# nlaha/genomics-rs

Measured on AMD Instinct MI355X. Metric: GCUPS (DP cell updates/s) at 30k×30k NW, 1/2/4/8 MI355X; % HBM roofline, higher is better.
Workload: dtype int16x2 (two pairs per register, exact, relative to int32 block bases)

## Files before the change

genomics-rs_amd/csrc/gx_api.h:

```cpp
#pragma once
#include <hip/hip_runtime.h>
#include <immintrin.h>

#include <algorithm>
#include <atomic>
#include <chrono>
#include <climits>
#include <condition_variable>
#include <functional>
#include <cstdio>
#include <cstdlib>
#include <cstring>
#include <memory>
#include <mutex>
#include <new>
#include <string>
#include <thread>
#include <vector>

#include "../../include/gx.h"
#include "gx_internal.h"

#pragma GCC visibility push(hidden)

// ... 206 lines not shown
    std::vector<DevBuf> free_list;
    std::vector<std::vector<uint8_t>> st_s1, st_s2;
    DevBuf st_chars;
    std::vector<size_t> st_off1, st_off2;
    SmallAlpha st_alpha;
    std::vector<Walk> walk_cache;
    TbOut tb_cache;
    PinnedBuf tb_pin;
    PinnedBuf io_pin;
    WorkPool workers;
    struct Slot {
        PinnedBuf fpin, tjpin, tbpin;
        hipEvent_t fb = nullptr, fe = nullptr, tb = nullptr, te = nullptr, fdone = nullptr, tdone = nullptr;
        hipEvent_t fres = nullptr;
        DevBuf held_pres;
        TbOut out;
        DevBuf held[4];
        void* tjob = nullptr;
        size_t tjob_cap = 0;
        std::vector<TbDev> tjob_last;
        void* fdesc = nullptr;
        size_t fdesc_cap = 0;
        std::vector<char> fdesc_last;
    } slots[4];
    int last_lay = 0, last_W = 0, last_pbytes = 0;
    int last_pbits = 0;
    int last_chunks = 1;
    int last_twin = 0;
    int last_rows = 0;
    int last_tbl = 0;
    int last_groups = 1;
    DevBuf sums_dev;
    unsigned long long* sums_dst = nullptr;
    std::vector<uint64_t> sums_host;
    bool pass_rec = false;
    size_t pass_off = 0, pass_P = 0;
    int pass_k = 0;
    std::vector<gx_result> pass_res;
    std::shared_ptr<struct KeptFill> kept;
    bool keep_capture = false;
    HostScores kept_hs{};
    Scores32 kept_sc{};
    uint64_t cmp_gpu = 0, cmp_host = 0, cmp_ovf = 0, cmp_levels = 0;
    uint64_t cmp_batches = 0;
    uint64_t cmp_cells = 0;
    double cmp_run_ms = 0.0;
    uint64_t suf_rounds = 0, suf_passes = 0;
    uint64_t suf_digit_passes[8] = {};
    double suf_sort_ms = 0.0, suf_lcp_ms = 0.0, suf_fold_ms = 0.0;
    uint64_t srch_words = 0;
    double srch_ms = 0.0, srch_locate_ms = 0.0;
};

struct PairHost {
// ... 8 lines not shown
    bool lcs_rows = false;
    size_t ltrace_off = 0, ltrace_bytes = 0;
    bool pairs_borrowed = false;
    bool pres_held = false;
    std::vector<PairDev> pd;
    std::vector<PairRes> res;
    int W = 4;
    int lay = 0;
    int slot = -1;
    PairRes* pin_res = nullptr;
    int* pin_status = nullptr;
    int total_bands = 0, total_strips = 0;
    bool planes_on = false, lcs_on = false, track_on = false;
    bool d8 = false;
    bool shift = false;
    bool twin = false;
    int rows = kRowsPerLane;
    bool w16 = false;
    bool nocodes = false;
    bool noskel = false;
    bool local_on = false;
    hipStream_t stream = nullptr;
    bool plan_only = false;
    bool table = false;
    int g = 0;
    double fill_ms = 0.0;
    bool wide = false;
    DevBuf wrows, wdesc, wres_d;
    std::vector<WideDev> wd;
    std::vector<WideRes> wres;
};

inline int job_strip_rows(const FillJob& j) { return j.twin && j.lay == 0 ? kWave * j.rows : strip_rows(j.lay); }

struct KeptFill {
    gx_context* ctx = nullptr;
    FillJob job;
    std::vector<int> dev_of;
    ~KeptFill();
};

static size_t align_up(size_t x, size_t a) { return (x + a - 1) / a * a; }


struct gx_table {
    gx_context* ctx = nullptr;
// ... 122 lines not shown
int run_fill_wide(gx_context* ctx, const std::vector<std::pair<const uint8_t*, const uint8_t*>>& proc,
                  const std::vector<PairHost>& ph, const HostScores& hs, int is_local, bool planes, bool track,
                  bool lcs, FillJob& job);
hipError_t enqueue_plane_sums(gx_context* ctx, const FillJob& job, const Scores32& sc,
                              unsigned long long* out, hipStream_t st = nullptr);

StartIn start_in(const FillJob& job, size_t p);
StartIn start_in(const PairRes& r);
int label_boundary(const HostScores& hs, int is_local, const uint8_t* s1, size_t n, const uint8_t* s2,
                   size_t m, uint64_t i, uint64_t j, int last, Walk& w);
int label_walk_records(const HostScores& hs, int is_local, const uint8_t* s1, size_t n, const uint8_t* s2,
                       size_t m, uint64_t si, uint64_t sj, const TbOut& tb, size_t p, Walk& w);
int run_traceback(gx_context* ctx, const std::vector<const FillJob*>& jv, const std::vector<TbStart>& starts,
                  TbOut& out, int slot, bool collect, bool dev_end_E, hipStream_t ts);
int run_traceback(gx_context* ctx, const FillJob& job, const std::vector<TbStart>& starts, TbOut& out,
                  int slot = -1, bool collect = true, bool dev_end_E = false);
int tb_collect(gx_context* ctx, int slot, size_t P, TbOut& out);
int start_cell_common(const HostScores& hs, int is_local, size_t n, size_t m, const StartIn& r,
                      uint64_t* si, uint64_t* sj, int64_t* score);
int copy_steps(const Walk& w, gx_step* steps, size_t cap);
int label_batch(gx_context* ctx, const std::vector<PairHost>& ph, const HostScores& hs, int is_local, bool track,
                const std::vector<int>& dev_of, const std::vector<uint64_t>& si,
                const std::vector<uint64_t>& sj, const std::vector<int64_t>& score,
                const std::vector<PairRes>& res, const TbOut& tb, double fill_ms, std::vector<Walk>& walks);

int batch_core_wide(gx_context* ctx, const std::vector<PairHost>& ph,
                    const std::vector<std::pair<const uint8_t*, const uint8_t*>>& proc, const HostScores& hs,
                    int is_local, bool planes, bool track, std::vector<Walk>& walks, double* fill_ms);
int batch_core_steps(gx_context* ctx, const std::vector<PairHost>& ph,
                     const std::vector<std::pair<const uint8_t*, const uint8_t*>>& proc, const HostScores& hs,
                     const Scores32& sc, int is_local, bool planes, bool track, int nsteps,
                     std::vector<Walk>& walks, double* fill_ms, const uint8_t* chars_dev,
                     const std::vector<size_t>* off1, const std::vector<size_t>* off2,
                     const SmallAlpha* staged_alpha, const PassSet* alt = nullptr);

struct SufInfo {
    uint64_t rounds = 0, passes = 0;
    uint64_t digit_passes[8] = {};
    double sort_ms = 0, lcp_ms = 0, fold_ms = 0;
};
struct SufDev {
    DevBuf text, k[2], v[2], rank, flags, table, tmp, small, fold, bwt;
    int cur = 0;
    uint64_t h = 8;
    uint64_t* pin = nullptr;
    void release(gx_context* ctx) {
        for (DevBuf* b : {&text, &k[0], &k[1], &v[0], &v[1], &rank, &flags, &table, &tmp, &small, &fold, &bwt})
            pool_put(ctx, *b);
    }
};
int suffix_device_sa(gx_context* ctx, const uint8_t* t, uint32_t N, bool with_stats, bool with_bwt, SufDev& w,
// ... 52 lines not shown
```

genomics-rs_amd/csrc/gx_api_batch.cpp:

```cpp
#include "gx_api.h"

int batch_core_wide(gx_context* ctx, const std::vector<PairHost>& ph,
                    const std::vector<std::pair<const uint8_t*, const uint8_t*>>& proc, const HostScores& hs,
                    int is_local, bool planes, bool track, std::vector<Walk>& walks, double* fill_ms) {
    const size_t P = ph.size();
    std::vector<size_t> idx;
    for (size_t p = 0; p < P; ++p) if (ph[p].n >= 1 && ph[p].m >= 1) idx.push_back(p);
    std::vector<PairHost> dph;
    std::vector<std::pair<const uint8_t*, const uint8_t*>> dproc;
    for (size_t p : idx) { dph.push_back(ph[p]); dproc.push_back(proc[p]); }
    FillJob job;
    std::vector<PairRes> res(P, PairRes{});
    std::vector<StartIn> sin(P, StartIn{0, 0, 0, 0});
    std::vector<uint64_t> si(P), sj(P);
    std::vector<int64_t> score(P);
    TbOut& tb = ctx->tb_cache;
    tb.ms = 0;
    int rc = GX_OK;
    if (!idx.empty()) {
        rc = run_fill_wide(ctx, dproc, dph, hs, is_local, planes, track, false, job);
        if (rc) { job_release(ctx, job); return rc; }
        for (size_t k = 0; k < idx.size(); ++k) { res[idx[k]] = job.res[k]; sin[idx[k]] = start_in(job, k); }
    }
    for (size_t p = 0; p < P; ++p) start_cell_common(hs, is_local, ph[p].n, ph[p].m, sin[p], &si[p], &sj[p], &score[p]);
// ... 77 lines not shown
        for (size_t k = 0; k < idx.size(); ++k) kdev[idx[k]] = (int)k;
        keep_job(ctx, job, kdev);
    }
    struct PhaseLog {
        clk::time_point c0, c1, c2;
        double fill_ms, tb_ms;
        size_t P;
        ~PhaseLog() {
            const char* e = getenv("GX_LOG");
            if (!e || strcmp(e, "debug")) return;
            auto ms = [](clk::time_point a, clk::time_point b) {
                return std::chrono::duration<double, std::milli>(b - a).count();
            };
            fprintf(stderr, "[gx DEBUG] batch P=%zu fill %.3f ms (kernel %.3f) traceback %.3f ms (kernel %.3f) "
                            "label %.3f ms\n", P, ms(c0, c1), fill_ms, ms(c1, c2), tb_ms, ms(c2, clk::now()));
        }
    } plog{c0, c1, c2, job.fill_ms, tb.ms, P};
    std::vector<int> dev_of(P, -1);
    for (size_t k = 0; k < idx.size(); ++k) dev_of[idx[k]] = (int)k;
    return label_batch(ctx, ph, hs, is_local, track, dev_of, si, sj, score, res, tb, job.fill_ms, walks);
}

static constexpr int kOverlapNo = -1000;
static int batch_core_overlap(gx_context* ctx, const std::vector<PairHost>& ph,
                              const std::vector<std::pair<const uint8_t*, const uint8_t*>>& proc, const HostScores& hs,
                              const Scores32& sc, int is_local, bool planes, int nsteps, std::vector<Walk>& walks, double* fill_ms,
                              const uint8_t* chars_dev, const std::vector<size_t>* off1,
                              const std::vector<size_t>* off2, const SmallAlpha& alpha,
                              const std::vector<size_t>& idx, const PassSet* alt) {
    const size_t P = ph.size(), Q = idx.size();
    size_t G = std::max<size_t>(2, (is_local ? Q / 5 : (Q + 1) / 2) & ~(size_t)1);
    if (const char* e = getenv("GX_OVERLAP_A"); e && atoi(e) >= 2 && (size_t)atoi(e) + 2 <= Q)
        G = (size_t)atoi(e) & ~(size_t)1;
    std::vector<size_t> gi[2];
    gi[0].assign(idx.begin(), idx.begin() + (long)G);
    gi[1].assign(idx.begin() + (long)G, idx.end());
    const std::vector<PairHost>* const PH[2] = {&ph, alt ? alt->ph : &ph};
    const std::vector<std::pair<const uint8_t*, const uint8_t*>>* const PR[2] = {&proc, alt ? alt->proc : &proc};
    const std::vector<size_t>* const O1[2] = {off1, alt ? alt->off1 : off1};
    const std::vector<size_t>* const O2[2] = {off2, alt ? alt->off2 : off2};
    std::vector<Walk>* const WK[2] = {&walks, alt ? alt->walks : &walks};
    const size_t poff[2] = {ctx->pass_off, alt ? alt->pass_off : ctx->pass_off};
    std::vector<PairHost> dph[2][2];
    std::vector<std::pair<const uint8_t*, const uint8_t*>> dproc[2][2];
    std::vector<size_t> o1[2][2], o2[2][2];
    for (int v = 0; v < 2; ++v)
// ... 22 lines not shown
    auto fill = [&](int g, int k) {
        FillJob& j = g == 0 ? jA[k & 1] : jB;
        j.stream = g == 0 ? sA : sB;
        const int v = k & 1;
        return run_fill(ctx, dproc[v][g], dph[v][g], sc, is_local, planes, false, false, j, chars_dev,
                        chars_dev ? &o1[v][g] : nullptr, chars_dev ? &o2[v][g] : nullptr, &alpha, 2 * g + (k & 1), false);
    };
    auto trace = [&](int k) {
        HIPCHK(hipStreamWaitEvent(sT, ctx->slots[k & 1].fdone, 0));
        HIPCHK(hipStreamWaitEvent(sT, ctx->slots[2 + (k & 1)].fdone, 0));
        return run_traceback(ctx, std::vector<const FillJob*>{&jA[k & 1], &jB}, starts, ctx->slots[k & 1].out, k & 1,
                             false, is_local != 0, sT);
    };
    auto take = [&](const FillJob& j, const std::vector<size_t>& g) {
        for (size_t q = 0; q < g.size(); ++q) res[g[q]] = j.res[q];
    };
    auto drain = [&]() {
        (void)hipStreamSynchronize(sA); (void)hipStreamSynchronize(sB); (void)hipStreamSynchronize(sT);
        (void)hipStreamSynchronize(ctx->cstream);
        for (auto& j : jA) job_release(ctx, j);
        job_release(ctx, jB);
        release_slots(ctx);
    };
    {
        FillJob pa, pb;
        pa.plan_only = pb.plan_only = true;
        int prc = run_fill(ctx, dproc[0][0], dph[0][0], sc, is_local, planes, false, false, pa, chars_dev,
                           chars_dev ? &o1[0][0] : nullptr, chars_dev ? &o2[0][0] : nullptr, &alpha, 0, false);
        if (!prc)
            prc = run_fill(ctx, dproc[0][1], dph[0][1], sc, is_local, planes, false, false, pb, chars_dev,
                           chars_dev ? &o1[0][1] : nullptr, chars_dev ? &o2[0][1] : nullptr, &alpha, 2, false);
        if (prc || !(pa.noskel && pb.noskel && pa.twin && pb.twin && pa.lay == pb.lay && pa.rows == pb.rows)) return kOverlapNo;
    }
    unsigned long long* const sums0 = ctx->sums_dst;
    HIPCHK(hipEventRecord(ctx->ev0, sA));
    int rc = fill(0, 0);
    if (!rc) { rc = fill(1, 0); jb_live = !rc; }
    if (!rc && !(jA[0].noskel && jB.noskel && jA[0].lay == jB.lay && jA[0].twin && jB.twin && jA[0].rows == jB.rows)) {
        drain();
        ctx->sums_dst = sums0;
        return kOverlapNo;
    }
    if (!rc) rc = trace(0);
    for (int k = 0; k < nsteps && !rc; ++k) {
        const int a = k & 1;
        if (k + 1 < nsteps) {
            if ((rc = fill(0, k + 1))) break;
            if ((rc = fill_collect(ctx, jB))) break;
            take(jB, gi[1]);
            job_release(ctx, jB);
            HIPCHK(hipStreamWaitEvent(sB, ctx->slots[a].te, 0));
            if ((rc = fill(1, k + 1))) break;
            if (k + 2 == nsteps) {
                HIPCHK(hipStreamWaitEvent(sB, ctx->slots[(k + 1) & 1].fdone, 0));
                HIPCHK(hipEventRecord(ctx->ev1, sB));
            }
            if (!(jA[(k + 1) & 1].noskel && jB.noskel)) { rc = fail(GX_EHIP, "overlapped batch: fill formats changed"); break; }
// ... 4 lines not shown
        }
        if ((rc = fill_collect(ctx, jA[a]))) break;
        take(jA[a], gi[0]);
        if (k + 1 == nsteps) {
            HIPCHK(hipEventSynchronize(ctx->ev1));
            float ms = 0.f;
            HIPCHK(hipEventElapsedTime(&ms, ctx->ev0, ctx->ev1));
            fsum = ms;
        }
        if ((rc = tb_collect(ctx, a, Q, ctx->slots[a].out))) break;
        job_release(ctx, jA[a]);
        for (size_t p = 0; p < P; ++p)
            start_cell_common(hs, is_local, ph[p].n, ph[p].m, start_in(res[p]), &si[p], &sj[p], &score[p]);
        ctx->pass_off = poff[a];
        if ((rc = label_batch(ctx, *PH[a], hs, is_local, false, dev_of, si, sj, score, res, ctx->slots[a].out,
                              jA[a].fill_ms + jB.fill_ms, *WK[a])))
            break;
    }
    drain();
    (void)jb_live;
    ctx->pass_off = poff[0];
    if (rc) return rc;
    ctx->last_groups = 2;
    if (fill_ms) *fill_ms = fsum / nsteps;
    return GX_OK;
}

int batch_core_steps(gx_context* ctx, const std::vector<PairHost>& ph,
                     const std::vector<std::pair<const uint8_t*, const uint8_t*>>& proc, const HostScores& hs,
                     const Scores32& sc, int is_local, bool planes, bool track, int nsteps,
                     std::vector<Walk>& walks, double* fill_ms, const uint8_t* chars_dev,
                     const std::vector<size_t>* off1, const std::vector<size_t>* off2,
                     const SmallAlpha* staged_alpha, const PassSet* alt) {
    const size_t P = ph.size();
    ctx->last_groups = 1;
    std::vector<size_t> idx;
    for (size_t p = 0; p < P; ++p) if (ph[p].n >= 1 && ph[p].m >= 1) idx.push_back(p);
    const std::vector<PairHost>* const PH[2] = {&ph, alt ? alt->ph : &ph};
    const std::vector<std::pair<const uint8_t*, const uint8_t*>>* const PR[2] = {&proc, alt ? alt->proc : &proc};
    const std::vector<size_t>* const O1[2] = {off1, alt ? alt->off1 : off1};
    const std::vector<size_t>* const O2[2] = {off2, alt ? alt->off2 : off2};
    std::vector<Walk>* const WK[2] = {&walks, alt ? alt->walks : &walks};
    const size_t poff[2] = {ctx->pass_off, alt ? alt->pass_off : ctx->pass_off};
    struct OffBack {
        gx_context* c;
        size_t v;
        ~OffBack() { c->pass_off = v; }
    } off_back{ctx, poff[0]};
    if (nsteps <= 1 || idx.empty() || getenv("GX_TRACE_FILE")) {
        double f = 0, fsum = 0;
        for (int s = 0; s < std::max(nsteps, 1); ++s) {
            const int v = s & 1;
            ctx->pass_off = poff[v];
            const int rc = batch_core(ctx, *PH[v], *PR[v], hs, sc, is_local, planes, track, *WK[v], &f, chars_dev,
                                      O1[v], O2[v], staged_alpha);
            if (rc) return rc;
            fsum += f;
        }
// ... 302 lines not shown
```

genomics-rs_amd/csrc/gx_api_context.cpp:

```cpp
#include "gx_api.h"


thread_local std::string g_err;
int fail(int code, const std::string& msg) {
    g_err = msg;
    return code;
}

int gx_internal_fail(int code, const std::string& msg) { return fail(code, msg); }

extern "C" const char* gx_last_error(void) { return g_err.c_str(); }
extern "C" const char* gx_version(void) { return "genomics-rs_amd 0.1 (gfx950)"; }

bool log_info() {
    static int v = -1;
    if (v < 0) {
        const char* e = getenv("GX_LOG");
        v = (e && (!strcmp(e, "info") || !strcmp(e, "debug"))) ? 1 : 0;
    }
    return v == 1;
}

void* pinned_grow(PinnedBuf& b, size_t bytes) {
    if (b.cap < bytes) {
// ... 143 lines not shown
        for (PinnedBuf* b : {&s.fpin, &s.tjpin, &s.tbpin})
            if (b->p) (void)hipHostFree(b->p);
        for (hipEvent_t e : {s.fb, s.fe, s.tb, s.te, s.fdone, s.tdone, s.fres})
            if (e) (void)hipEventDestroy(e);
        if (s.tjob) (void)hipFree(s.tjob);
        if (s.fdesc) (void)hipFree(s.fdesc);
    }
    if (ctx->ev0) (void)hipEventDestroy(ctx->ev0);
    if (ctx->ev1) (void)hipEventDestroy(ctx->ev1);
    if (ctx->ev2) (void)hipEventDestroy(ctx->ev2);
    if (ctx->stream) (void)hipStreamDestroy(ctx->stream);
    if (ctx->cstream) (void)hipStreamDestroy(ctx->cstream);
    if (ctx->stream2) (void)hipStreamDestroy(ctx->stream2);
    if (ctx->tstream) (void)hipStreamDestroy(ctx->tstream);
    if (ctx->pstream) (void)hipStreamDestroy(ctx->pstream);
    delete ctx;
}

void release_held(gx_context* ctx, int slot) {
    for (DevBuf& b : ctx->slots[slot].held) { pool_put(ctx, b); b = DevBuf{}; }
}
void release_slots(gx_context* ctx) {
    (void)hipStreamSynchronize(ctx->cstream);
    for (int k = 0; k < 4; ++k) {
        release_held(ctx, k);
        pool_put(ctx, ctx->slots[k].held_pres);
    }
}
```

genomics-rs_amd/csrc/gx_api_fill.cpp:

```cpp
#include "gx_api.h"

void unshift_results(FillJob& j) {
    if (!j.shift) return;
    for (size_t p = 0; p < j.res.size() && p < j.pd.size(); ++p)
        if (j.pd[p].n >= 1 && j.pd[p].m >= 1) j.res[p].end_SM += (j.pd[p].n + j.pd[p].m) * j.g;
}

void job_release(gx_context* ctx, FillJob& j) {
    if (j.pairs_borrowed) { j.pairs = DevBuf{}; j.pairs_borrowed = false; }
    if (j.pres_held) { j.pres = DevBuf{}; j.pres_held = false; }
    pool_put(ctx, j.chars); pool_put(ctx, j.planes); pool_put(ctx, j.codes); pool_put(ctx, j.feed);
    pool_put(ctx, j.progress); pool_put(ctx, j.sres); pool_put(ctx, j.pres); pool_put(ctx, j.pairs);
    pool_put(ctx, j.counter); pool_put(ctx, j.skel); pool_put(ctx, j.ccodes);
    pool_put(ctx, j.wrows); pool_put(ctx, j.wdesc); pool_put(ctx, j.wres_d); pool_put(ctx, j.lcs);
}

void release_or_hold(gx_context* ctx, FillJob& j, bool last_pass, bool* held) {
    if (ctx->keep_capture && last_pass) { *held = true; return; }
    job_release(ctx, j);
}
void keep_job(gx_context* ctx, FillJob& j, const std::vector<int>& dev_of) {
    auto k = std::make_shared<KeptFill>();
    k->ctx = ctx;
    k->dev_of = dev_of;
// ... 44 lines not shown
    if (twin && is_local) {
        const int K = std::max(0, -std::min(sc.sm, sc.smm));
        scl.koff = K; scl.sm = sc.sm + K; scl.smm = sc.smm + K;
    }
    const bool w16 = tp.w16;
    job.w16 = w16;
    job.nocodes = w16;
    job.noskel = job.nocodes;
    const int rows = tp.rows;
    job.rows = rows;
    const int SRf = twin ? kWave * rows : SR;
    const bool twin_tbl = twin && tbl && (!planes || w16) && scl.sm >= 0 && scl.sm <= 255 && scl.smm >= 0 &&
                          scl.smm <= 255;
    ctx->last_twin = twin ? 1 : 0;
    ctx->last_rows = twin ? rows : 0;
    ctx->last_tbl = (twin ? twin_tbl : tbl) ? 1 : 0;
    const int Wf = twin ? Wt : W;
    const size_t plane_esz = d8 ? 1 : sizeof(int32_t);
    job.W = Wf;
    ctx->last_lay = cs2 ? 2 : lay; ctx->last_W = Wf;
    ctx->last_pbytes = planes ? (w16 ? 2 : (int)(plane_esz * 3)) : 0;
    ctx->last_pbits = planes ? (w16 ? 12 : (int)(plane_esz * 24)) : 0;
    const size_t P = ph.size();
    if (job.plan_only) { job.twin = twin; return GX_OK; }
    job.pd.assign(P, PairDev{});
    size_t chars_bytes = 0, plane_elems = 0, code_elems = 0, feed_recs = 0, prog_elems = 0, skel_elems = 0;
    std::vector<size_t> c1o(P), c2o(P), po(P), co(P), fo(P), gofs(P), so(P);
    int bands = 0, strips = 0;
    std::vector<int> mate(P, -1), half(P, 0);
    if (twin)
        for (const auto& t : tw) {
            mate[t.first] = t.second; mate[t.second] = t.first;
            half[t.first] = 0;
            if (t.second != t.first) half[t.second] = 1;
        }
    for (size_t p = 0; p < P; ++p) {
        const int n = (int)ph[p].n, m = (int)ph[p].m;
        PairDev& d = job.pd[p];
        d.n = n; d.m = m;
        int ns = n, ms = m;
        if (twin) {
            const PairHost& y = ph[mate[p]];
            ns = (int)std::max(ph[p].n, y.n); ms = (int)std::max(ph[p].m, y.m);
        }
        d.strips = ceil_div(ns, SRf);
        d.bands = ceil_div(d.strips, Wf);
        d.rows = twin ? rows : 0;
// ... 12 lines not shown
        if (!twin) {
            d.band_base = bands;
            bands += d.bands;
            so[p] = skel_elems; skel_elems += (size_t)d.strips * d.skel_stride;
            fo[p] = feed_recs; feed_recs += (size_t)std::max(d.bands - 1, 0) * d.feed_stride;
            gofs[p] = prog_elems; prog_elems += (size_t)std::max(d.bands - 1, 0) * kProgStride;
        }
    }
    if (twin)
        for (const auto& t : tw) {
            PairDev& d = job.pd[t.first];
            const size_t a = t.first, b = t.second;
            d.band_base = bands; job.pd[b].band_base = bands;
            bands += d.bands;
            so[a] = so[b] = skel_elems; skel_elems += (size_t)d.strips * d.skel_stride;
            fo[a] = fo[b] = feed_recs; feed_recs += (size_t)std::max(d.bands - 1, 0) * d.feed_stride * 2;
            gofs[a] = gofs[b] = prog_elems; prog_elems += (size_t)std::max(d.bands - 1, 0) * kProgStride;
            if (w16) { po[a] = po[b] = plane_elems; plane_elems += (size_t)d.strips * d.t4 * w12_group_bytes(rows); }
        }
    job.total_bands = bands;
    job.total_strips = strips;
    int rc;
    const int nplanes = w16 ? 1 : (lcs && !job.lcs_rows) ? 4 : 3;
    if (!chars_dev) {
        if ((rc = pool_get(ctx, chars_bytes, &job.chars, fs))) return rc;
    }
    if (planes && (rc = pool_get(ctx, plane_elems * plane_esz * nplanes, &job.planes, fs))) return rc;
    const bool want_codes = codes && !job.nocodes;
    if (want_codes && (rc = pool_get(ctx, code_elems * sizeof(uint32_t), &job.codes, fs))) return rc;
    if ((rc = pool_get(ctx, std::max<size_t>(skel_elems, 1) * sizeof(int), &job.skel, fs))) return rc;
    if ((rc = pool_get(ctx, std::max<size_t>(feed_recs, 1) * sizeof(Rec), &job.feed, fs))) return rc;
    if ((rc = pool_get(ctx, std::max(strips, 1) * sizeof(StripRes), &job.sres, fs))) return rc;
    if (getenv("GX_LCS_ALONE"))
        HIPCHK(hipMemsetAsync(job.sres.p, 0, std::max(strips, 1) * sizeof(StripRes), fs));
    const size_t res_bytes = P * sizeof(PairRes), prog_bytes = std::max<size_t>(prog_elems, 1) * sizeof(int);
    if ((rc = pool_get(ctx, res_bytes + 64 + prog_bytes, &job.pres, fs))) return rc;
    int* const counter = (int*)((char*)job.pres.p + res_bytes);
    int* const progress = counter + 16;
    std::vector<int> order;
    order.reserve(2 * (size_t)bands);
    if (twin) {
        int maxb = 0;
        for (const auto& t : tw) maxb = std::max(maxb, job.pd[t.first].bands);
        for (int lb = 0; lb < maxb; ++lb)
            for (size_t q = 0; q < tw.size(); ++q)
                if (lb < job.pd[tw[q].first].bands) { order.push_back((int)q); order.push_back(lb); }
        for (const auto& t : tw) { order.push_back(t.first); order.push_back(t.second); }
    } else {
        int maxb = 0;
        for (size_t p = 0; p < P; ++p) maxb = std::max(maxb, job.pd[p].bands);
// ... 364 lines not shown
```

genomics-rs_amd/csrc/gx_api_walk.cpp:

```cpp
#include "gx_api.h"

StartIn start_in(const FillJob& job, size_t p) {
    if (job.wide) return StartIn{job.wres[p].end_SM, job.wres[p].lmax_val, (uint64_t)job.wres[p].lmax_i,
                                 (uint64_t)job.wres[p].lmax_j};
    const PairRes& r = job.res[p];
    return StartIn{r.end_SM, r.lmax_val, (uint64_t)r.lmax_i, (uint64_t)r.lmax_j};
}
StartIn start_in(const PairRes& r) { return StartIn{r.end_SM, r.lmax_val, (uint64_t)r.lmax_i, (uint64_t)r.lmax_j}; }

int label_boundary(const HostScores& hs, int is_local, const uint8_t* s1, size_t n, const uint8_t* s2,
                   size_t m, uint64_t i, uint64_t j, int last, Walk& w) {
    gx_result& r = w.res;
    for (;;) {
        int64_t I, D, S;
        boundary_cell(hs, i, j, &I, &D, &S);
        const int64_t mx = smax(I, S, D, is_local);
        gx_step st{};
        st.i = i; st.j = j;
        bool di, dj;
        if (mx == S) {
            const bool mt = tb_match(s1, n, s2, m, i, j);
            st.choice = mt ? GX_MATCH : GX_MISMATCH;
            if (mt) r.matches++; else r.mismatches++;
            last = st.choice;
// ... 265 lines not shown
    }
    for (uint64_t i = 1; i <= n; ++i) {
        int64_t I, D, S;
        boundary_cell(hs, i, 0, &I, &D, &S);
        consider(smax(I, S, D, 1), i, 0);
    }
    if (n >= 1 && m >= 1) consider(r.lmax_val, r.lmax_i, r.lmax_j);
    *si = bi; *sj = bj; *score = best;
    return GX_OK;
}

int copy_steps(const Walk& w, gx_step* steps, size_t cap) {
    if (!steps) return GX_OK;
    if (w.steps.size() > cap) return fail(GX_ECAP, "steps capacity " + std::to_string(cap) + " < " +
                                                       std::to_string(w.steps.size()));
    memcpy(steps, w.steps.data(), w.steps.size() * sizeof(gx_step));
    return GX_OK;
}


int label_batch(gx_context* ctx, const std::vector<PairHost>& ph, const HostScores& hs, int is_local, bool track,
                const std::vector<int>& dev_of, const std::vector<uint64_t>& si,
                const std::vector<uint64_t>& sj, const std::vector<int64_t>& score,
                const std::vector<PairRes>& res, const TbOut& tb, double fill_ms, std::vector<Walk>& walks) {
    const size_t P = ph.size();
    walks.resize(P);
    std::vector<int> prc(P, GX_OK);
    std::vector<std::string> perr(P);
    const std::function<void(size_t)> label_one = [&](size_t p) {
        if (dev_of[p] >= 0)
            prc[p] = label_walk_records(hs, is_local, ph[p].s1, ph[p].n, ph[p].s2, ph[p].m, si[p], sj[p], tb,
                                        (size_t)dev_of[p], walks[p]);
        else
            prc[p] = label_walk(hs, is_local, ph[p].s1, ph[p].n, ph[p].s2, ph[p].m, si[p], sj[p], 0,
                                MovesSrc{nullptr, 0}, walks[p]);
        if (prc[p]) perr[p] = g_err;
    };
    size_t cap = 16;
    if (const char* e = getenv("GX_LABEL_THREADS"); e && atoi(e) > 0) cap = (size_t)atoi(e);
    const size_t nthreads = std::min<size_t>({P, (size_t)std::max(1u, std::thread::hardware_concurrency()), cap});
    if (nthreads <= 1) {
        for (size_t p = 0; p < P; ++p) label_one(p);
    } else {
        ctx->workers.run(P, nthreads - 1, label_one);
    }
    for (size_t p = 0; p < P; ++p) {
        if (prc[p]) return fail(prc[p], perr[p]);
        Walk& w = walks[p];
        const bool interior = ph[p].n >= 1 && ph[p].m >= 1 && track;
        w.res.score = score[p];
        w.res.start_i = si[p]; w.res.start_j = sj[p];
        w.res.max_cell_i = interior ? (uint64_t)res[p].max_i : 0;
        w.res.max_cell_j = interior ? (uint64_t)res[p].max_j : 0;
        w.res.matches_at_max = interior ? (uint64_t)res[p].mam : 0;
        w.res.fill_us = (int64_t)(fill_ms * 1000.0);
        w.res.retrace_us = (int64_t)(tb.ms * 1000.0);
    }
    if (ctx->pass_rec) {
        const size_t base = (size_t)ctx->pass_k * ctx->pass_P + ctx->pass_off;
        if (base + P <= ctx->pass_res.size())
            for (size_t p = 0; p < P; ++p) ctx->pass_res[base + p] = walks[p].res;
        ++ctx->pass_k;
    }
    return GX_OK;
}
```

genomics-rs_amd/gxamd.py:

```python
from __future__ import annotations

import ctypes
import enum
import logging
import os
from dataclasses import dataclass, field
from typing import List, Optional, Sequence as Seq, Tuple

import numpy as np

_HERE = os.path.dirname(os.path.abspath(__file__))
_log = logging.getLogger("gxamd")
LIB_PATH = os.environ.get("GX_LIB", os.path.join(_HERE, "libgx_amd.so"))

GX_TABLE_PLANES = 1
GX_TABLE_MATCHES = 2
GX_ALIGN_MAX_CELL = 4
GX_STAGED_PLANE_SUMS = 8
GX_STAGED_ALTERNATE = 16
GX_STAGED_KEEP_PLANES = 32

_CODES = {0: "GX_OK", 1: "GX_EINVAL", 2: "GX_ESEQ", 3: "GX_ERANGE", 4: "GX_ENOMEM", 5: "GX_EHIP",
          6: "GX_EPANIC", 7: "GX_ECAP", 8: "GX_EIO", 9: "GX_EPARSE"}

# ... 27 lines not shown

class CSuffixStats(ctypes.Structure):
    _fields_ = [(k, ctypes.c_uint64) for k in ("num_internal", "num_leaves", "num_nodes", "string_depth_sum",
                                               "max_string_depth", "longest_repeat_start", "longest_repeat_len")]


class CResult(ctypes.Structure):
    _fields_ = [("score", ctypes.c_int64), ("matches", ctypes.c_uint64), ("mismatches", ctypes.c_uint64),
                ("gap_extensions", ctypes.c_uint64), ("opening_gaps", ctypes.c_uint64),
                ("n_steps", ctypes.c_uint64), ("start_i", ctypes.c_uint64), ("start_j", ctypes.c_uint64),
                ("max_cell_i", ctypes.c_uint64), ("max_cell_j", ctypes.c_uint64),
                ("matches_at_max", ctypes.c_uint64), ("fill_us", ctypes.c_int64), ("retrace_us", ctypes.c_int64)]


CELL_DTYPE = np.dtype([("insert_score", "<i8"), ("delete_score", "<i8"), ("sub_score", "<i8"),
                       ("insert_matches", "<u8"), ("delete_matches", "<u8"), ("sub_matches", "<u8")])
STEP_DTYPE = np.dtype([("choice", "u1"), ("pad", "u1", (7,)), ("i", "<u8"), ("j", "<u8")])

EXPORTED = ["gx_last_error", "gx_version", "gx_context_create", "gx_context_destroy", "gx_context_trim",
            "gx_alignment_table", "gx_table_info", "gx_table_export", "gx_table_export_plane", "gx_table_export_rows",
            "gx_table_plane_sums", "gx_retrace", "gx_table_free", "gx_align", "gx_align_batch", "gx_align_batch_multi",
            "gx_stage_pairs",
            "gx_run_staged", "gx_run_staged_steps", "gx_staged_plane_sums", "gx_staged_steps",
            "gx_staged_pass_results", "gx_fill_info", "gx_batch_chunks", "gx_fill_twin", "gx_fill_groups", "gx_fill_plane_bits", "gx_plane_bytes_per_cell", "gx_twin_admission",
            "gx_twin_admission_mode", "gx_twin_admission_rows", "gx_fill_rows", "gx_fill_score_table", "gx_plan_layout",
            "gx_plan_twin_rows", "gx_staged_table",
            "gx_fasta_load",
            "gx_config_load", "gx_format_alignment", "gx_format_table",
            "gx_common_substring_host", "gx_common_substring", "gx_compare_pair", "gx_compare_matrix",
            "gx_compare_info", "gx_compare_batches", "gx_compare_segment_height", "gx_compare_run_stats",
            "gx_common_substring_candidates_host",
            "gx_suffix_tree_stats", "gx_suffix_info", "gx_suffix_digit_passes", "gx_suffix_tile", "gx_format_suffix_stats",
            "gx_suffix_index_build", "gx_suffix_index_free", "gx_suffix_index_info", "gx_suffix_index_export",
            "gx_suffix_index_search", "gx_search_info"]

_lib = None


def lib():
    global _lib
    if _lib is not None:
        return _lib
    if not os.path.exists(LIB_PATH):
        raise GxError(5, f"{LIB_PATH} not built (run `make -C genomics-rs_amd` or __graft_entry__.build())")
    L = ctypes.CDLL(LIB_PATH)
    vp, sz, u8p = ctypes.c_void_p, ctypes.c_size_t, ctypes.POINTER(ctypes.c_uint8)
    L.gx_last_error.restype = ctypes.c_char_p
# ... 10 lines not shown
    L.gx_table_export_rows.argtypes = [vp, ctypes.c_int, sz, sz, vp, sz]
    L.gx_table_plane_sums.argtypes = [vp, vp]
    L.gx_staged_plane_sums.argtypes = [vp, vp, sz, ctypes.POINTER(sz)]
    L.gx_staged_steps.argtypes = [vp, sz, vp, sz, ctypes.POINTER(sz)]
    L.gx_staged_pass_results.argtypes = [vp, vp, sz, ctypes.POINTER(sz)]
    L.gx_retrace.argtypes = [vp, ctypes.c_int, vp, sz, ctypes.POINTER(CResult)]
    L.gx_table_free.argtypes = [vp]
    L.gx_table_free.restype = None
    L.gx_align.argtypes = [vp, vp, sz, vp, sz, ctypes.POINTER(CScores), ctypes.c_int, ctypes.c_int,
                           ctypes.c_uint32, vp, sz, ctypes.POINTER(CResult)]
    L.gx_align_batch.argtypes = [vp, vp, vp, vp, vp, sz, ctypes.POINTER(CScores), ctypes.c_int, ctypes.c_uint32,
                                 vp, vp, vp]
    L.gx_align_batch_multi.argtypes = [vp, ctypes.c_int, vp, vp, vp, vp, sz, ctypes.POINTER(CScores), ctypes.c_int,
                                       ctypes.c_uint32, vp, vp, vp]
    L.gx_stage_pairs.argtypes = [vp, vp, vp, vp, vp, sz]
    L.gx_run_staged.argtypes = [vp, ctypes.POINTER(CScores), ctypes.c_int, ctypes.c_int, ctypes.c_uint32, vp,
                                ctypes.POINTER(ctypes.c_double)]
    L.gx_run_staged_steps.argtypes = [vp, ctypes.POINTER(CScores), ctypes.c_int, ctypes.c_int, ctypes.c_uint32,
                                      ctypes.c_int, vp, ctypes.POINTER(ctypes.c_double)]
    L.gx_fill_info.argtypes = [vp] + [ctypes.POINTER(ctypes.c_int)] * 3
    L.gx_batch_chunks.argtypes = [vp]
    L.gx_fill_twin.argtypes = [vp]
    L.gx_fill_groups.argtypes = [vp]
    if hasattr(L, "gx_fill_plane_bits"):
        L.gx_fill_plane_bits.argtypes = [vp]
    L.gx_plane_bytes_per_cell.argtypes = [ctypes.POINTER(CScores), ctypes.c_int]
    L.gx_twin_admission.argtypes = [ctypes.POINTER(CScores), ctypes.c_int, ctypes.c_int64,
                                    ctypes.POINTER(ctypes.c_int64)]
    L.gx_twin_admission_mode.argtypes = [ctypes.POINTER(CScores), ctypes.c_int, ctypes.c_int, ctypes.c_int64,
                                         ctypes.POINTER(ctypes.c_int64)]
    if hasattr(L, "gx_twin_admission_rows"):
        L.gx_twin_admission_rows.argtypes = [ctypes.POINTER(CScores), ctypes.c_int, ctypes.c_int, ctypes.c_int64,
                                             ctypes.c_int, ctypes.POINTER(ctypes.c_int64)]
        L.gx_fill_rows.argtypes = [vp]
    if hasattr(L, "gx_fill_score_table"):
        L.gx_fill_score_table.argtypes = [vp]
        L.gx_plan_twin_rows.argtypes = [ctypes.POINTER(CScores), ctypes.POINTER(ctypes.c_int64),
                                        ctypes.POINTER(ctypes.c_int64), sz, ctypes.c_int,
                                        ctypes.POINTER(ctypes.c_int)]
    L.gx_staged_table.argtypes = [vp, sz, ctypes.POINTER(vp)]
    L.gx_plan_layout.argtypes = [ctypes.POINTER(CScores), ctypes.c_int, ctypes.POINTER(ctypes.c_int64),
                                 ctypes.POINTER(ctypes.c_int64), sz, ctypes.c_int, ctypes.c_int]
    L.gx_fasta_load.argtypes = [ctypes.c_char_p, vp, sz, vp, vp, vp, vp, sz, ctypes.POINTER(sz), ctypes.POINTER(sz)]
    L.gx_config_load.argtypes = [ctypes.c_char_p, ctypes.POINTER(CScores)]
    L.gx_format_alignment.argtypes = [vp, sz, vp, sz, vp, sz, ctypes.POINTER(CResult), vp, sz, ctypes.POINTER(sz)]
    L.gx_format_table.argtypes = [vp, sz, vp, sz, vp, sz, vp, vp, vp, ctypes.c_int, vp, sz, ctypes.POINTER(sz)]
# ... 202 lines not shown
        _check(lib().gx_context_create(device, ctypes.byref(p)))
        self.ptr = p
        self.device = device

    def close(self):
        if self.ptr:
            lib().gx_context_destroy(self.ptr)
            self.ptr = None

    def trim(self):
        _check(lib().gx_context_trim(self.ptr))

    def fill_info(self) -> dict:
        v = [ctypes.c_int() for _ in range(3)]
        _check(lib().gx_fill_info(self.ptr, *[ctypes.byref(x) for x in v]))
        bits = lib().gx_fill_plane_bits(self.ptr) if hasattr(lib(), "gx_fill_plane_bits") else 8 * v[2].value
        return {"layout": v[0].value, "band_waves": v[1].value,
                "plane_bytes_per_cell": bits // 8 if bits % 8 == 0 else bits / 8,
                "chunks": lib().gx_batch_chunks(self.ptr), "twin": lib().gx_fill_twin(self.ptr),
                "groups": lib().gx_fill_groups(self.ptr),
                "twin_rows": lib().gx_fill_rows(self.ptr) if hasattr(lib(), "gx_fill_rows") else 2,
                "score_table": lib().gx_fill_score_table(self.ptr) if hasattr(lib(), "gx_fill_score_table") else -1}

    def __del__(self):
        try:
            self.close()
        except Exception:
            pass


_default_ctx: dict = {}


def device_for_rank(local_rank: int) -> int:
    dm = os.environ.get("GX_DEVICE_MAP", "")
    devs = [int(x) for x in dm.split(",") if x.strip()]
    return devs[local_rank % len(devs)] if devs else local_rank


def default_context(device: Optional[int] = None) -> Context:
    if device is None:
        device = device_for_rank(int(os.environ.get("LOCAL_RANK", "0"))) if "GX_DEVICE" not in os.environ \
            else int(os.environ["GX_DEVICE"])
    if device not in _default_ctx:
        _default_ctx[device] = Context(device)
    return _default_ctx[device]


class AlignmentTable:

    def __init__(self, ptr, s1: bytes, s2: bytes, flags: int):
# ... 605 lines not shown
```

include/gx.h:

```cpp
#ifndef GX_H
#define GX_H

#include <stddef.h>
#include <stdint.h>

#ifdef __cplusplus
extern "C" {
#endif

#define GX_OK 0
#define GX_EINVAL 1
#define GX_ESEQ 2
#define GX_ERANGE 3
#define GX_ENOMEM 4
#define GX_EHIP 5
#define GX_EPANIC 6
#define GX_ECAP 7
#define GX_EIO 8
#define GX_EPARSE 9

typedef struct gx_scores {
    int64_t s_match;
    int64_t s_mismatch;
    int64_t g;
// ... 86 lines not shown
                         int is_local, uint32_t flags, gx_step* const* steps, const size_t* caps, gx_result* out);

int gx_stage_pairs(gx_context* ctx, const uint8_t* const* s1, const size_t* n, const uint8_t* const* s2,
                   const size_t* m, size_t npairs);
int gx_run_staged(gx_context* ctx, const gx_scores* scores, int is_local, int keep_planes, uint32_t flags,
                  gx_result* out, double* fill_ms_out);
int gx_run_staged_steps(gx_context* ctx, const gx_scores* scores, int is_local, int keep_planes, uint32_t flags,
                        int nsteps, gx_result* out, double* fill_ms_out);
#define GX_STAGED_PLANE_SUMS 8u
int gx_staged_plane_sums(const gx_context* ctx, uint64_t* out, size_t cap, size_t* n_values);
#define GX_STAGED_ALTERNATE 16u
#define GX_STAGED_KEEP_PLANES 32u
int gx_staged_table(gx_context* ctx, size_t pair, gx_table** table_out);
int gx_staged_steps(const gx_context* ctx, size_t pair, gx_step* steps, size_t cap, size_t* n_steps);
int gx_staged_pass_results(const gx_context* ctx, gx_result* out, size_t cap, size_t* n_values);
int gx_fill_info(const gx_context* ctx, int* layout, int* band_waves, int* plane_bytes_per_cell);
int gx_fill_plane_bits(const gx_context* ctx);
int gx_batch_chunks(const gx_context* ctx);
int gx_fill_twin(const gx_context* ctx);
int gx_fill_rows(const gx_context* ctx);
int gx_fill_score_table(const gx_context* ctx);

int gx_fill_groups(const gx_context* ctx);
int gx_plane_bytes_per_cell(const gx_scores* scores, int is_local);

int gx_twin_admission(const gx_scores* scores, int band_waves, int64_t col_gap, int64_t* bound);
int gx_twin_admission_mode(const gx_scores* scores, int is_local, int band_waves, int64_t col_gap, int64_t* bound);
int gx_twin_admission_rows(const gx_scores* scores, int is_local, int band_waves, int64_t col_gap,
                           int rows_per_lane, int64_t* bound);
int gx_plan_twin_rows(const gx_scores* scores, const int64_t* n, const int64_t* m, size_t npairs, int grid_cap,
                      int* band_waves);
int gx_plan_layout(const gx_scores* scores, int is_local, const int64_t* n, const int64_t* m, size_t npairs,
                   int track, int grid_cap);

int gx_fasta_load(const char* path, uint8_t* buf, size_t cap, uint64_t* name_off, uint64_t* name_len,
                  uint64_t* seq_off, uint64_t* seq_len, size_t rec_cap, size_t* n_records, size_t* bytes_needed);
int gx_config_load(const char* path, gx_scores* out);

int gx_format_alignment(const uint8_t* s1, size_t n, const uint8_t* s2, size_t m, const gx_step* steps,
                        size_t n_steps, const gx_result* res, char* out, size_t cap, size_t* needed);

int gx_format_table(const uint8_t* s1, size_t n, const uint8_t* s2, size_t m, const gx_step* steps, size_t n_steps,
                    const int64_t* insert_plane, const int64_t* delete_plane, const int64_t* sub_plane, int color,
                    char* out, size_t cap, size_t* needed);


// ... 51 lines not shown
```

Measured before the change: 3328.

## Rotate three fill jobs across six traceback slots to deepen fill/traceback overlap

Adds a rotating overlap scheme for global two-group batches. Three fill jobs cycle across four fill slots and six walk slots on two fill streams plus a traceback stream, with host collection and labelling lagging three steps behind. The goal is to keep the GPU busy while the host collects and labels earlier batches, instead of draining between pairs of fills. Plane buffers are sized to a common floor so pooled allocations can be reused across rotations, at the cost of more live device memory and more complex event dependencies.

```diff
diff --git a/genomics-rs_amd/csrc/gx_api.h b/genomics-rs_amd/csrc/gx_api.h
--- a/genomics-rs_amd/csrc/gx_api.h
+++ b/genomics-rs_amd/csrc/gx_api.h
@@ -252,7 +252,7 @@
         void* fdesc = nullptr;
         size_t fdesc_cap = 0;
         std::vector<char> fdesc_last;
-    } slots[4];
+    } slots[6];
     int last_lay = 0, last_W = 0, last_pbytes = 0;
     int last_pbits = 0;
     int last_chunks = 1;
@@ -260,6 +260,7 @@
     int last_rows = 0;
     int last_tbl = 0;
     int last_groups = 1;
+    int last_scheme = 0;
     DevBuf sums_dev;
     unsigned long long* sums_dst = nullptr;
     std::vector<uint64_t> sums_host;
@@ -314,6 +315,8 @@
     bool local_on = false;
     hipStream_t stream = nullptr;
     bool plan_only = false;
+    size_t plane_bytes = 0;
+    size_t plane_floor = 0;
     bool table = false;
     int g = 0;
     double fill_ms = 0.0;
@@ -482,11 +485,22 @@
 int label_batch(gx_context* ctx, const std::vector<PairHost>& ph, const HostScores& hs, int is_local, bool track,
                 const std::vector<int>& dev_of, const std::vector<uint64_t>& si,
                 const std::vector<uint64_t>& sj, const std::vector<int64_t>& score,
-                const std::vector<PairRes>& res, const TbOut& tb, double fill_ms, std::vector<Walk>& walks);
+                const std::vector<PairRes>& res, const TbOut& tb, double fill_ms, std::vector<Walk>& walks,
+                const std::vector<const TbOut*>* tb_of = nullptr);
 
 int batch_core_wide(gx_context* ctx, const std::vector<PairHost>& ph,
                     const std::vector<std::pair<const uint8_t*, const uint8_t*>>& proc, const HostScores& hs,
                     int is_local, bool planes, bool track, std::vector<Walk>& walks, double* fill_ms);
+struct RotatePlan {
+    int job;
+    int fslot;
+    int wslot;
+    int stream;
+    int wait_walk;
+    int collected;
+    int labelled;
+};
+RotatePlan overlap_rotate_plan(int i);
 int batch_core_steps(gx_context* ctx, const std::vector<PairHost>& ph,
                      const std::vector<std::pair<const uint8_t*, const uint8_t*>>& proc, const HostScores& hs,
                      const Scores32& sc, int is_local, bool planes, bool track, int nsteps,
diff --git a/genomics-rs_amd/csrc/gx_api_batch.cpp b/genomics-rs_amd/csrc/gx_api_batch.cpp
--- a/genomics-rs_amd/csrc/gx_api_batch.cpp
+++ b/genomics-rs_amd/csrc/gx_api_batch.cpp
@@ -123,6 +123,27 @@
 }
 
 static constexpr int kOverlapNo = -1000;
+
+RotatePlan overlap_rotate_plan(int i) {
+    RotatePlan r;
+    r.job = i % 3;
+    r.fslot = 2 * (i & 1) + ((i >> 1) & 1);
+    r.wslot = i % 6;
+    r.stream = i & 1;
+    r.wait_walk = i >= 3 ? i - 3 : -1;
+    r.collected = i >= 3 ? i - 3 : -1;
+    r.labelled = i >= 5 ? 2 * ((i - 5) / 2) + 1 : -1;
+    return r;
+}
+extern "C" int gx_overlap_rotate_plan(int fill, int* out7) {
+    if (fill < 0 || !out7) return fail(GX_EINVAL, "gx_overlap_rotate_plan: fill < 0 or out is NULL");
+    const RotatePlan r = overlap_rotate_plan(fill);
+    const int v[7] = {r.job, r.fslot, r.wslot, r.stream, r.wait_walk, r.collected, r.labelled};
+    std::copy(v, v + 7, out7);
+    return GX_OK;
+}
+extern "C" int gx_overlap_scheme(const gx_context* ctx) { return ctx ? ctx->last_scheme : -1; }
+
 static int batch_core_overlap(gx_context* ctx, const std::vector<PairHost>& ph,
                               const std::vector<std::pair<const uint8_t*, const uint8_t*>>& proc, const HostScores& hs,
                               const Scores32& sc, int is_local, bool planes, int nsteps, std::vector<Walk>& walks, double* fill_ms,
@@ -191,8 +212,8 @@
         job_release(ctx, jB);
         release_slots(ctx);
     };
+    FillJob pa, pb;
     {
-        FillJob pa, pb;
         pa.plan_only = pb.plan_only = true;
         int prc = run_fill(ctx, dproc[0][0], dph[0][0], sc, is_local, planes, false, false, pa, chars_dev,
                            chars_dev ? &o1[0][0] : nullptr, chars_dev ? &o2[0][0] : nullptr, &alpha, 0, false);
@@ -202,6 +223,99 @@
         if (prc || !(pa.noskel && pb.noskel && pa.twin && pb.twin && pa.lay == pb.lay && pa.rows == pb.rows)) return kOverlapNo;
     }
     unsigned long long* const sums0 = ctx->sums_dst;
+    const char* rot_e = getenv("GX_OVERLAP_ROTATE");
+    if (!is_local && G == std::max<size_t>(2, ((Q + 1) / 2) & ~(size_t)1) && !(rot_e && !strcmp(rot_e, "0"))) {
+        FillJob jobs[3];
+        for (FillJob& j : jobs) j.plane_floor = std::max(pa.plane_bytes, pb.plane_bytes);
+        const int N = 2 * nsteps;
+        std::vector<TbStart> gstarts[2];
+        std::vector<int> gdev(P, -1);
+        for (int g = 0; g < 2; ++g)
+            for (size_t q = 0; q < gi[g].size(); ++q) {
+                gstarts[g].push_back(TbStart{(int)dph[0][g][q].n, (int)dph[0][g][q].m, 0});
+                gdev[gi[g][q]] = (int)q;
+            }
+        std::vector<const TbOut*> tb_of(P, nullptr);
+        double fms[6] = {0, 0, 0, 0, 0, 0};
+        auto drain_r = [&]() {
+            (void)hipStreamSynchronize(sA); (void)hipStreamSynchronize(sB); (void)hipStreamSynchronize(sT);
+            (void)hipStreamSynchronize(ctx->cstream);
+            for (auto& j : jobs) job_release(ctx, j);
+            release_slots(ctx);
+        };
+        auto enqueue = [&](int i) -> int {
+            const RotatePlan rp = overlap_rotate_plan(i);
+            const int g = i & 1, v = (i >> 1) & 1;
+            FillJob& j = jobs[rp.job];
+            hipStream_t const fs = rp.stream ? sB : sA;
+            if (i == 0) HIPCHK(hipEventRecord(ctx->ev0, fs));
+#ifndef GX_MUT_NO_ROTATE_WAIT
+            if (rp.wait_walk >= 0) HIPCHK(hipStreamWaitEvent(fs, ctx->slots[overlap_rotate_plan(rp.wait_walk).wslot].te, 0));
+#endif
+            j.stream = fs;
+            int r = run_fill(ctx, dproc[v][g], dph[v][g], sc, is_local, planes, false, false, j, chars_dev,
+                             chars_dev ? &o1[v][g] : nullptr, chars_dev ? &o2[v][g] : nullptr, &alpha, rp.fslot, false);
+            if (r) return r;
+            if (!(j.noskel && j.twin && j.lay == pa.lay && j.rows == pa.rows))
+                return i < 2 ? kOverlapNo : fail(GX_EHIP, "overlapped batch: fill formats changed");
+            if (i == N - 1) {
+                HIPCHK(hipStreamWaitEvent(fs, ctx->slots[overlap_rotate_plan(i - 1).fslot].fdone, 0));
+                HIPCHK(hipEventRecord(ctx->ev1, fs));
+            }
+            HIPCHK(hipStreamWaitEvent(sT, ctx->slots[rp.fslot].fdone, 0));
+            return run_traceback(ctx, std::vector<const FillJob*>{&j}, gstarts[g], ctx->slots[rp.wslot].out, rp.wslot,
+                                 false, false, sT);
+        };
+        auto collect = [&](int i) -> int {
+            const RotatePlan rp = overlap_rotate_plan(i);
+            FillJob& j = jobs[rp.job];
+            const int r = fill_collect(ctx, j);
+            if (r) return r;
+            fms[rp.wslot] = j.fill_ms;
+            take(j, gi[i & 1]);
+            job_release(ctx, j);
+            return GX_OK;
+        };
+        auto label = [&](int k) -> int {
+            const int a = k & 1;
+            for (int g = 0; g < 2; ++g) {
+                const int ws = overlap_rotate_plan(2 * k + g).wslot;
+                const int r = tb_collect(ctx, ws, gi[g].size(), ctx->slots[ws].out);
+                if (r) return r;
+                for (size_t p : gi[g]) tb_of[p] = &ctx->slots[ws].out;
+            }
+            for (size_t p = 0; p < P; ++p)
+                start_cell_common(hs, is_local, ph[p].n, ph[p].m, start_in(res[p]), &si[p], &sj[p], &score[p]);
+            ctx->pass_off = poff[a];
+            const int w0 = overlap_rotate_plan(2 * k).wslot, w1 = overlap_rotate_plan(2 * k + 1).wslot;
+            return label_batch(ctx, *PH[a], hs, is_local, false, gdev, si, sj, score, res, ctx->slots[w0].out,
+                               fms[w0] + fms[w1], *WK[a], &tb_of);
+        };
+        int rc = GX_OK;
+        for (int t = 0; t < N + 3 && !rc; ++t) {
+            if (t >= 3) rc = collect(t - 3);
+            if (!rc && t < N) rc = enqueue(t);
+            if (!rc && t >= 3 && ((t - 3) & 1)) rc = label((t - 3) / 2);
+        }
+        if (!rc) {
+            auto span = [&]() -> int {
+                HIPCHK(hipEventSynchronize(ctx->ev1));
+                float ms = 0.f;
+                HIPCHK(hipEventElapsedTime(&ms, ctx->ev0, ctx->ev1));
+                fsum = ms;
+                return GX_OK;
+            };
+            rc = span();
+        }
+        drain_r();
+        ctx->pass_off = poff[0];
+        if (rc == kOverlapNo) ctx->sums_dst = sums0;
+        if (rc) return rc;
+        ctx->last_groups = 2;
+        ctx->last_scheme = 2;
+        if (fill_ms) *fill_ms = fsum / nsteps;
+        return GX_OK;
+    }
     HIPCHK(hipEventRecord(ctx->ev0, sA));
     int rc = fill(0, 0);
     if (!rc) { rc = fill(1, 0); jb_live = !rc; }
@@ -252,6 +366,7 @@
     ctx->pass_off = poff[0];
     if (rc) return rc;
     ctx->last_groups = 2;
+    ctx->last_scheme = 1;
     if (fill_ms) *fill_ms = fsum / nsteps;
     return GX_OK;
 }
@@ -264,6 +379,7 @@
                      const SmallAlpha* staged_alpha, const PassSet* alt) {
     const size_t P = ph.size();
     ctx->last_groups = 1;
+    ctx->last_scheme = 0;
     std::vector<size_t> idx;
     for (size_t p = 0; p < P; ++p) if (ph[p].n >= 1 && ph[p].m >= 1) idx.push_back(p);
     const std::vector<PairHost>* const PH[2] = {&ph, alt ? alt->ph : &ph};
diff --git a/genomics-rs_amd/csrc/gx_api_context.cpp b/genomics-rs_amd/csrc/gx_api_context.cpp
--- a/genomics-rs_amd/csrc/gx_api_context.cpp
+++ b/genomics-rs_amd/csrc/gx_api_context.cpp
@@ -189,7 +189,7 @@
 }
 void release_slots(gx_context* ctx) {
     (void)hipStreamSynchronize(ctx->cstream);
-    for (int k = 0; k < 4; ++k) {
+    for (int k = 0; k < (int)(sizeof ctx->slots / sizeof ctx->slots[0]); ++k) {
         release_held(ctx, k);
         pool_put(ctx, ctx->slots[k].held_pres);
     }
diff --git a/genomics-rs_amd/csrc/gx_api_fill.cpp b/genomics-rs_amd/csrc/gx_api_fill.cpp
--- a/genomics-rs_amd/csrc/gx_api_fill.cpp
+++ b/genomics-rs_amd/csrc/gx_api_fill.cpp
@@ -90,7 +90,6 @@
     ctx->last_pbytes = planes ? (w16 ? 2 : (int)(plane_esz * 3)) : 0;
     ctx->last_pbits = planes ? (w16 ? 12 : (int)(plane_esz * 24)) : 0;
     const size_t P = ph.size();
-    if (job.plan_only) { job.twin = twin; return GX_OK; }
     job.pd.assign(P, PairDev{});
     size_t chars_bytes = 0, plane_elems = 0, code_elems = 0, feed_recs = 0, prog_elems = 0, skel_elems = 0;
     std::vector<size_t> c1o(P), c2o(P), po(P), co(P), fo(P), gofs(P), so(P);
@@ -149,10 +148,12 @@
     job.total_strips = strips;
     int rc;
     const int nplanes = w16 ? 1 : (lcs && !job.lcs_rows) ? 4 : 3;
+    job.plane_bytes = planes ? plane_elems * plane_esz * nplanes : 0;
+    if (job.plan_only) { job.pd.clear(); return GX_OK; }
     if (!chars_dev) {
         if ((rc = pool_get(ctx, chars_bytes, &job.chars, fs))) return rc;
     }
-    if (planes && (rc = pool_get(ctx, plane_elems * plane_esz * nplanes, &job.planes, fs))) return rc;
+    if (planes && (rc = pool_get(ctx, std::max(job.plane_bytes, job.plane_floor), &job.planes, fs))) return rc;
     const bool want_codes = codes && !job.nocodes;
     if (want_codes && (rc = pool_get(ctx, code_elems * sizeof(uint32_t), &job.codes, fs))) return rc;
     if ((rc = pool_get(ctx, std::max<size_t>(skel_elems, 1) * sizeof(int), &job.skel, fs))) return rc;
diff --git a/genomics-rs_amd/csrc/gx_api_walk.cpp b/genomics-rs_amd/csrc/gx_api_walk.cpp
--- a/genomics-rs_amd/csrc/gx_api_walk.cpp
+++ b/genomics-rs_amd/csrc/gx_api_walk.cpp
@@ -311,14 +311,16 @@
 int label_batch(gx_context* ctx, const std::vector<PairHost>& ph, const HostScores& hs, int is_local, bool track,
                 const std::vector<int>& dev_of, const std::vector<uint64_t>& si,
                 const std::vector<uint64_t>& sj, const std::vector<int64_t>& score,
-                const std::vector<PairRes>& res, const TbOut& tb, double fill_ms, std::vector<Walk>& walks) {
+                const std::vector<PairRes>& res, const TbOut& tb, double fill_ms, std::vector<Walk>& walks,
+                const std::vector<const TbOut*>* tb_of) {
     const size_t P = ph.size();
     walks.resize(P);
     std::vector<int> prc(P, GX_OK);
     std::vector<std::string> perr(P);
+    auto tb_for = [&](size_t p) -> const TbOut& { return tb_of && (*tb_of)[p] ? *(*tb_of)[p] : tb; };
     const std::function<void(size_t)> label_one = [&](size_t p) {
         if (dev_of[p] >= 0)
-            prc[p] = label_walk_records(hs, is_local, ph[p].s1, ph[p].n, ph[p].s2, ph[p].m, si[p], sj[p], tb,
+            prc[p] = label_walk_records(hs, is_local, ph[p].s1, ph[p].n, ph[p].s2, ph[p].m, si[p], sj[p], tb_for(p),
                                         (size_t)dev_of[p], walks[p]);
         else
             prc[p] = label_walk(hs, is_local, ph[p].s1, ph[p].n, ph[p].s2, ph[p].m, si[p], sj[p], 0,
@@ -343,7 +345,7 @@
         w.res.max_cell_j = interior ? (uint64_t)res[p].max_j : 0;
         w.res.matches_at_max = interior ? (uint64_t)res[p].mam : 0;
         w.res.fill_us = (int64_t)(fill_ms * 1000.0);
-        w.res.retrace_us = (int64_t)(tb.ms * 1000.0);
+        w.res.retrace_us = (int64_t)(tb_for(p).ms * 1000.0);
     }
     if (ctx->pass_rec) {
         const size_t base = (size_t)ctx->pass_k * ctx->pass_P + ctx->pass_off;
diff --git a/genomics-rs_amd/gxamd.py b/genomics-rs_amd/gxamd.py
--- a/genomics-rs_amd/gxamd.py
+++ b/genomics-rs_amd/gxamd.py
@@ -73,7 +73,7 @@
             "gx_table_plane_sums", "gx_retrace", "gx_table_free", "gx_align", "gx_align_batch", "gx_align_batch_multi",
             "gx_stage_pairs",
             "gx_run_staged", "gx_run_staged_steps", "gx_staged_plane_sums", "gx_staged_steps",
-            "gx_staged_pass_results", "gx_fill_info", "gx_batch_chunks", "gx_fill_twin", "gx_fill_groups", "gx_fill_plane_bits", "gx_plane_bytes_per_cell", "gx_twin_admission",
+            "gx_staged_pass_results", "gx_fill_info", "gx_batch_chunks", "gx_fill_twin", "gx_fill_groups", "gx_overlap_scheme", "gx_overlap_rotate_plan", "gx_fill_plane_bits", "gx_plane_bytes_per_cell", "gx_twin_admission",
             "gx_twin_admission_mode", "gx_twin_admission_rows", "gx_fill_rows", "gx_fill_score_table", "gx_plan_layout",
             "gx_plan_twin_rows", "gx_staged_table",
             "gx_fasta_load",
@@ -130,6 +130,9 @@
     L.gx_batch_chunks.argtypes = [vp]
     L.gx_fill_twin.argtypes = [vp]
     L.gx_fill_groups.argtypes = [vp]
+    if hasattr(L, "gx_overlap_scheme"):
+        L.gx_overlap_scheme.argtypes = [vp]
+        L.gx_overlap_rotate_plan.argtypes = [ctypes.c_int, ctypes.POINTER(ctypes.c_int)]
     if hasattr(L, "gx_fill_plane_bits"):
         L.gx_fill_plane_bits.argtypes = [vp]
     L.gx_plane_bytes_per_cell.argtypes = [ctypes.POINTER(CScores), ctypes.c_int]
@@ -378,11 +381,23 @@
                 "twin_rows": lib().gx_fill_rows(self.ptr) if hasattr(lib(), "gx_fill_rows") else 2,
                 "score_table": lib().gx_fill_score_table(self.ptr) if hasattr(lib(), "gx_fill_score_table") else -1}
 
+    def overlap_scheme(self) -> int:
+        return lib().gx_overlap_scheme(self.ptr)
+
     def __del__(self):
         try:
             self.close()
         except Exception:
             pass
+
+
+ROTATE_PLAN_FIELDS = ("job", "fslot", "wslot", "stream", "wait_walk", "collected", "labelled")
+
+
+def overlap_rotate_plan(fill: int) -> dict:
+    v = (ctypes.c_int * 7)()
+    _check(lib().gx_overlap_rotate_plan(fill, v))
+    return dict(zip(ROTATE_PLAN_FIELDS, (int(x) for x in v)))
 
 
 _default_ctx: dict = {}
diff --git a/include/gx.h b/include/gx.h
--- a/include/gx.h
+++ b/include/gx.h
@@ -132,6 +132,8 @@
 int gx_fill_score_table(const gx_context* ctx);
 
 int gx_fill_groups(const gx_context* ctx);
+int gx_overlap_scheme(const gx_context* ctx);
+int gx_overlap_rotate_plan(int fill, int* out7);
 int gx_plane_bytes_per_cell(const gx_scores* scores, int is_local);
 
 int gx_twin_admission(const gx_scores* scores, int band_waves, int64_t col_gap, int64_t* bound);
```

After: 3574 (median of 6 runs). 1.07x the previous value.
